# Desperodoo/distributed_multi_agent_reinforcement_learning

Measured on AMD Instinct MI355X. Metric: env-steps/sec (whole node), pursuit-evasion 8-agent 4096-env, higher is better.
Workload: dtype f64 environment / f32 policy (f32 matrix products evaluated from exact 3-way bf16 operand splits, f32 accumulation and storage)

## Files before the change

### distributed_multi_agent_reinforcement_learning_amd/csrc/mappo_ops.hip

```cpp
#include <hip/hip_runtime.h>
#include <stdint.h>
#include <stdlib.h>
#include <string.h>

#include <mutex>

#include "mappo_ops.h"
#include "mappo_ops_diag.h"
#include "sb_common.hpp"

namespace {

constexpr int MAX_P = 16;

__device__ __forceinline__ float msg_dot4(const float *w, const float4 &qv) {
    return __builtin_fmaf(w[3], qv.w, __builtin_fmaf(w[2], qv.z, __builtin_fmaf(w[1], qv.y, w[0] * qv.x)));
}

struct MsgDims {
    int R, P, K, E, din, q_div, adj_mode, rpb;
    int64_t p_rs, q_rs, e_rs, adj_rs, o_is;
};

__device__ __forceinline__ float rl_f(float v, int lane) { return __int_as_float(__builtin_amdgcn_readlane(__float_as_int(v), lane)); }
__device__ __forceinline__ uint32_t rl_u(uint32_t v, int lane) { return (uint32_t)__builtin_amdgcn_readlane((int)v, lane); }

struct MsgRow {
    float vp, ve, vq;
    uint32_t va0, va1;
    int kv;
};

template <bool QS, bool AS>
__device__ __forceinline__ MsgRow msgw_load(const MsgDims &d, int r, const float *__restrict__ p, const float *__restrict__ q,
                                            const float *__restrict__ e, const void *__restrict__ adj, const int32_t *__restrict__ kvalid,
                                            bool use_kvalid) {
    const int lane = threadIdx.x & 63, qr = r / d.q_div;
    MsgRow m;
    m.vp = lane < 4 * d.P ? p[(size_t)r * d.p_rs + lane] : 0.f;
    m.ve = (d.din == 8 && lane < 4) ? e[(size_t)r * d.e_rs + lane] : 0.f;
    m.vq = 0.f;
    if (QS) m.vq = lane < 4 * d.K ? q[(size_t)qr * d.q_rs + lane] : 0.f;
    m.va0 = m.va1 = 0u;
    if (AS) {
        if (d.adj_mode == MO_ADJ_TENSOR) {
            m.va0 = lane < d.P * d.K ? __float_as_uint(((const float *)adj)[(size_t)r * d.adj_rs + lane]) : 0u;
        } else if (d.adj_mode == MO_ADJ_BITS) {
            const uint32_t *bw = (const uint32_t *)adj + (size_t)r * d.adj_rs;
            const int n = d.P * MO_ADJ_ROW_WORDS(d.K);
            m.va0 = lane < n ? bw[lane] : 0u;
            m.va1 = lane + 64 < n ? bw[lane + 64] : 0u;
        }
    }
    m.kv = use_kvalid ? kvalid[qr] : d.K;
    return m;
}

template <bool QS>
__device__ __forceinline__ float4 msgw_q(const MsgRow &m, const float4 *__restrict__ q4, int j) {
    if (QS) return make_float4(rl_f(m.vq, 4 * j), rl_f(m.vq, 4 * j + 1), rl_f(m.vq, 4 * j + 2), rl_f(m.vq, 4 * j + 3));
    return q4[j];
}
template <bool AS>
__device__ __forceinline__ uint32_t msgw_word(const MsgRow &m, const uint32_t *__restrict__ bw, int idx) {
    if (AS) return idx < 64 ? rl_u(m.va0, idx) : rl_u(m.va1, idx - 64);
    return bw[idx];
}

struct MsgMask { uint64_t nz, col; bool zero_one; };
__device__ __forceinline__ MsgMask msgw_mask(const MsgRow &m, int P, int K) {
    const float a = __uint_as_float(m.va0);
    MsgMask k;
    k.nz = __ballot(a != 0.f);
    k.zero_one = __ballot(a != 0.f && a != 1.f) == 0ull;
    k.col = 0ull;
    for (int i = 0; i < P; i++) k.col |= 1ull << (i * K);
    return k;
}
__device__ __forceinline__ float msgw_row_norm(const MsgRow &m, const MsgMask &k, int i, int K) {
    if (k.zero_one) return (float)__popcll((k.nz >> (i * K)) & ((K >= 64) ? ~0ull : ((1ull << K) - 1ull)));
    float s = 0.f;
    for (int j = 0; j < K; j++) s += fabsf(__uint_as_float(rl_u(m.va0, i * K + j)));
    return s;
}

template <int EV>
struct FV {
    float v[EV];
    __device__ __forceinline__ FV() {}
    __device__ __forceinline__ FV(float s) {
#pragma unroll
        for (int e = 0; e < EV; e++) v[e] = s;
// ... 1671 lines not shown
    constexpr int U = 4;
    const int wave = threadIdx.x >> 6, lane = threadIdx.x & 63;
    const int i = lane & 15, kk = lane >> 4;
    const int m0 = blockIdx.y * 128 * AM + (wave >> 1) * 64 * AM, n0 = blockIdx.z * 128 * BN + (wave & 1) * 64 * BN;
    const int64_t steps = K >> 2;
    const int64_t s_beg = steps * blockIdx.x / gridDim.x, s_end = steps * (blockIdx.x + 1) / gridDim.x;
    const int64_t lda4 = 4 * lda, ldb4 = 4 * ldb;
    const float *pa = A + (4 * s_beg + kk) * lda + m0 + 4 * i;
    const float *pb = B + (4 * s_beg + kk) * ldb + n0 + 4 * i;
    v4f acc[AM][4][BN][4];
#pragma unroll
    for (int a = 0; a < AM; a++)
#pragma unroll
        for (int t = 0; t < 4; t++)
#pragma unroll
            for (int b = 0; b < BN; b++)
#pragma unroll
                for (int v = 0; v < 4; v++) acc[a][t][b][v] = (v4f){0.f, 0.f, 0.f, 0.f};
    const int64_t n_s = s_end - s_beg, pairs = n_s / (2 * U);
    WgradRegs<AM, BN, U> r0, r1;
    if (pairs > 0) wgrad_load<AM, BN, U>(r0, pa, pb, lda4, ldb4);
    for (int64_t c = 0; c < pairs; c++) {
        wgrad_load<AM, BN, U>(r1, pa + U * lda4, pb + U * ldb4, lda4, ldb4);
        __builtin_amdgcn_sched_barrier(0);
        wgrad_mma<AM, BN, U>(r0, acc);
        __builtin_amdgcn_sched_barrier(0);
        const int64_t adv = (c + 1 < pairs) ? 2 * U : U;
        pa += adv * lda4;
        pb += adv * ldb4;
        wgrad_load<AM, BN, U>(r0, pa, pb, lda4, ldb4);
        __builtin_amdgcn_sched_barrier(0);
        wgrad_mma<AM, BN, U>(r1, acc);
        __builtin_amdgcn_sched_barrier(0);
    }
    {
        pa = A + (4 * (s_beg + pairs * 2 * U) + kk) * lda + m0 + 4 * i;
        pb = B + (4 * (s_beg + pairs * 2 * U) + kk) * ldb + n0 + 4 * i;
        WgradRegs<AM, BN, 1> r;
        for (int64_t s = s_beg + pairs * 2 * U; s < s_end; s++) {
            wgrad_load<AM, BN, 1>(r, pa, pb, lda4, ldb4);
            wgrad_mma<AM, BN, 1>(r, acc);
            pa += lda4;
            pb += ldb4;
        }
        if (blockIdx.x == gridDim.x - 1 && (K & 3)) {
            const bool live = 4 * steps + kk < K;
#pragma unroll
            for (int a = 0; a < AM; a++) r.a[0][a] = live ? *(const float4 *)(pa + a * 64) : make_float4(0.f, 0.f, 0.f, 0.f);
#pragma unroll
            for (int b = 0; b < BN; b++) r.b[0][b] = live ? *(const float4 *)(pb + b * 64) : make_float4(0.f, 0.f, 0.f, 0.f);
            wgrad_mma<AM, BN, 1>(r, acc);
        }
    }
    float *po = part + ((size_t)blockIdx.x * M + m0 + 16 * kk) * N + n0 + 4 * i;
#pragma unroll
    for (int a = 0; a < AM; a++)
#pragma unroll
        for (int t = 0; t < 4; t++)
#pragma unroll
            for (int q = 0; q < 4; q++)
#pragma unroll
                for (int b = 0; b < BN; b++)
                    *(float4 *)(po + (size_t)(64 * a + 4 * q + t) * N + 64 * b) =
                        make_float4(acc[a][t][b][0][q], acc[a][t][b][1][q], acc[a][t][b][2][q], acc[a][t][b][3][q]);
}

__global__ __launch_bounds__(256) void k_wgrad_reduce(int S, int MN, const float *__restrict__ part, float *__restrict__ C, int accumulate) {
    __shared__ float sm[4][64];
    const int q = threadIdx.x >> 6, lane = threadIdx.x & 63;
    const int idx = blockIdx.x * 64 + lane;
    float s = 0.f;
    if (idx < MN) {
#pragma unroll 8
        for (int x = q; x < S; x += 4) s += part[(size_t)x * MN + idx];
    }
    sm[q][lane] = s;
    __syncthreads();
    if (q == 0 && idx < MN) {
        const float t = (sm[0][lane] + sm[1][lane]) + (sm[2][lane] + sm[3][lane]);
        C[idx] = accumulate ? C[idx] + t : t;
    }
}

constexpr int SB_DEPTH = 4;

template <int MT, int NT>
struct SbWgCfg {
    static constexpr int M = 128 * MT, N = 128 * NT, COLS = M + N, FQ = COLS / 4;
    static constexpr int CR = 16, NO = 2;
    static constexpr int WGM = MT >= NT ? 4 : 2;
    static constexpr int WGN = 8 / WGM;
    static constexpr int TM = M / 32 / WGM, TN = N / 32 / WGN;
    static constexpr int UNITS = 2 * NO * FQ;
    static constexpr int IMG = 3 * NO * COLS;
    static constexpr int LDS_BYTES = 2 * IMG * 16;
};

__device__ __forceinline__ int sb_swz(int f) { return (f & ~3) | ((f & 3) ^ ((f >> 3) & 3)); }
template <int MT, int NT>
__global__ __launch_bounds__(512) void k_sb_wgrad(const float *__restrict__ A, int64_t lda, const float *__restrict__ B, int64_t ldb, int64_t K,
                                                  float *__restrict__ part, const float *__restrict__ A2, int64_t lda2, int M1) {
    using C = SbWgCfg<MT, NT>;
    extern __shared__ uint4 sb_lds[];
    const int tid = threadIdx.x, lane = tid & 63, wave = tid >> 6;
    const int i = lane & 31, g = lane >> 5;
    const bool on = tid < C::UNITS;
    const int rest = on ? tid / C::FQ : 0, col = 4 * (tid % C::FQ);
    const int row_in_chunk = 4 * rest;
    const bool in_a2 = A2 != nullptr && col >= M1 && col < C::M;
    const int64_t ld = in_a2 ? lda2 : (col < C::M ? lda : ldb);
    const float *src = (in_a2 ? A2 + (col - M1) : (col < C::M ? A + col : B + (col - C::M))) + row_in_chunk * ld;
    const int slot2 = 2 * ((rest >> 1) * C::COLS + col) + (rest & 1), sx = (col >> 3) & 3;
    const int wm = wave / C::WGN, wn = wave % C::WGN;
    const int64_t chunks = K / C::CR;
    const int64_t c_beg = chunks * blockIdx.x / gridDim.x, c_end = chunks * (blockIdx.x + 1) / gridDim.x;

    f32x16 acc[C::TM][C::TN];
#pragma unroll
    for (int a = 0; a < C::TM; a++)
#pragma unroll
        for (int b = 0; b < C::TN; b++)
#pragma unroll
            for (int r = 0; r < 16; r++) acc[a][b][r] = 0.f;

    float4 raw[SB_DEPTH][4];
    auto fetch = [&](float4 (&r)[4], int64_t c) {
        if (!on || c >= c_end) return;
        const float *p = src + c * C::CR * ld;
#pragma unroll
        for (int j = 0; j < 4; j++) r[j] = *(const float4 *)(p + j * ld);
    };
    auto stage = [&](const float4 (&r)[4], uint4 *img) {
        if (!on) return;
        uint2 *img2 = (uint2 *)img;
#pragma unroll
        for (int t = 0; t < 4; t++) {
            uint32_t p[3][2];
#pragma unroll
            for (int q = 0; q < 2; q++) {
                const float x0 = t == 0 ? r[2 * q].x : t == 1 ? r[2 * q].y : t == 2 ? r[2 * q].z : r[2 * q].w;
                const float x1 = t == 0 ? r[2 * q + 1].x : t == 1 ? r[2 * q + 1].y : t == 2 ? r[2 * q + 1].z : r[2 * q + 1].w;
                sb_split2(x0, x1, p[0][q], p[1][q], p[2][q]);
            }
#pragma unroll
            for (int s = 0; s < 3; s++) img2[2 * s * C::NO * C::COLS + slot2 + 2 * (t ^ sx)] = make_uint2(p[s][0], p[s][1]);
        }
    };
    auto multiply = [&](const uint4 *buf) {
        const uint4 *img = buf + g * C::COLS;
        constexpr int PS = C::NO * C::COLS;
        if constexpr (C::TN <= C::TM) {
            uint4 b[C::TN][3];
#pragma unroll
            for (int nt = 0; nt < C::TN; nt++) {
                const int f = sb_swz(C::M + 32 * (wn * C::TN + nt) + i);
#pragma unroll
                for (int s = 0; s < 3; s++) b[nt][s] = img[s * PS + f];
            }
#pragma unroll
            for (int mt = 0; mt < C::TM; mt++) {
                const int f = sb_swz(32 * (wm * C::TM + mt) + i);
                uint4 a[3];
#pragma unroll
                for (int s = 0; s < 3; s++) a[s] = img[s * PS + f];
#pragma unroll
                for (int nt = 0; nt < C::TN; nt++) acc[mt][nt] = sb_mma6_32(a, b[nt], acc[mt][nt]);
            }
        } else {
            uint4 a[C::TM][3];
#pragma unroll
            for (int mt = 0; mt < C::TM; mt++) {
                const int f = sb_swz(32 * (wm * C::TM + mt) + i);
#pragma unroll
                for (int s = 0; s < 3; s++) a[mt][s] = img[s * PS + f];
            }
#pragma unroll
            for (int nt = 0; nt < C::TN; nt++) {
                const int f = sb_swz(C::M + 32 * (wn * C::TN + nt) + i);
                uint4 b[3];
#pragma unroll
                for (int s = 0; s < 3; s++) b[s] = img[s * PS + f];
#pragma unroll
                for (int mt = 0; mt < C::TM; mt++) acc[mt][nt] = sb_mma6_32(a[mt], b, acc[mt][nt]);
            }
        }
    };
#pragma unroll
    for (int d = 0; d < SB_DEPTH; d++) fetch(raw[d], c_beg + d);
    if (c_beg < c_end) {
        stage(raw[0], sb_lds);
        fetch(raw[0], c_beg + SB_DEPTH);
    }
    lds_barrier();
    for (int64_t c = c_beg; c < c_end; c += SB_DEPTH) {
#pragma unroll
        for (int d = 0; d < SB_DEPTH; d++) {
            const int64_t cc = c + d;
            if (cc >= c_end) break;
            uint4 *cur = sb_lds + (d & 1) * C::IMG, *nxt = sb_lds + ((d + 1) & 1) * C::IMG;
            if (wave < 4) {
                if (cc + 1 < c_end) stage(raw[(d + 1) % SB_DEPTH], nxt);
                fetch(raw[(d + 1) % SB_DEPTH], cc + 1 + SB_DEPTH);
                multiply(cur);
            } else {
                multiply(cur);
                if (cc + 1 < c_end) stage(raw[(d + 1) % SB_DEPTH], nxt);
                fetch(raw[(d + 1) % SB_DEPTH], cc + 1 + SB_DEPTH);
            }
            lds_barrier();
        }
    }
    if (blockIdx.x == gridDim.x - 1 && (K % C::CR)) {
        float4 r[4];
#pragma unroll
        for (int j = 0; j < 4; j++)
            r[j] = (on && chunks * C::CR + row_in_chunk + j < K) ? *(const float4 *)(src + (chunks * C::CR + j) * ld) : make_float4(0.f, 0.f, 0.f, 0.f);
        stage(r, sb_lds);
        lds_barrier();
        multiply(sb_lds);
    }
    float *po = part + (size_t)blockIdx.x * C::M * C::N + (size_t)(32 * wm * C::TM + 4 * g) * C::N + 32 * wn * C::TN + i;
#pragma unroll
    for (int mt = 0; mt < C::TM; mt++)
#pragma unroll
        for (int r = 0; r < 16; r++)
#pragma unroll
            for (int nt = 0; nt < C::TN; nt++) po[(size_t)(32 * mt + 8 * (r / 4) + (r % 4)) * C::N + 32 * nt] = acc[mt][nt][r];
}


struct NbrArgs {
    int R, P, E, T, relu;
    int64_t za_es, za_ts, zc_es, zc_ts;
    int64_t adj_rs;
    int64_t out_ld;
};
struct NbrJobs { mo_nbr_job j[MO_NBR_MAX_JOBS]; };
template <int PT>
__global__ void k_nbr_mean(NbrArgs a, NbrJobs jobs, const float *__restrict__ adj) {
    const mo_nbr_job &job = jobs.j[blockIdx.y];
    const float *__restrict__ za = job.z_actor, *__restrict__ zc = job.z_critic, *__restrict__ bias = job.bias;
    float *__restrict__ out_a = job.out_actor, *__restrict__ out_c = job.out_critic;
    const int P = a.P, E = a.E, f = threadIdx.x, lane = threadIdx.x & 63;
    const float bf = bias ? bias[f] : 0.f;
    const float inv_p = 1.f / fmaxf((float)P, 1e-12f);
    for (int r = blockIdx.x; r < a.R; r += gridDim.x) {
        const int n = r / a.T, t = r - n * a.T;
        if (out_a) {
            const float *zr = za + (size_t)n * a.za_es + (size_t)t * a.za_ts;
            float z[PT];
#pragma unroll
            for (int j = 0; j < PT; j++) z[j] = j < P ? zr[(size_t)j * E + f] : 0.f;
            float w = 0.f;
            if (P * P <= 64) {
                const float av = lane < P * P ? adj[(size_t)r * a.adj_rs + lane] : 0.f;
                const int li = lane / P < P ? lane / P : P - 1;
                float nrm = 0.f;
                for (int j = 0; j < P; j++) nrm += fabsf(__shfl(av, li * P + j));
                w = av / fmaxf(nrm, 1e-12f);
            }
#pragma unroll
            for (int i = 0; i < PT; i++)
                if (i < P) {
                    float acc = 0.f;
                    if (P * P <= 64) {
#pragma unroll
                        for (int j = 0; j < PT; j++)
                            if (j < P) acc = __builtin_fmaf(rl_f(w, i * P + j), z[j], acc);
                    } else {
                        const float *ar = adj + (size_t)r * a.adj_rs + (size_t)i * P;
                        float nrm = 0.f;
                        for (int j = 0; j < P; j++) nrm += fabsf(ar[j]);
                        nrm = fmaxf(nrm, 1e-12f);
#pragma unroll
                        for (int j = 0; j < PT; j++)
                            if (j < P) acc = __builtin_fmaf(ar[j] / nrm, z[j], acc);
                    }
                    acc += bf;
                    out_a[((size_t)r * P + i) * a.out_ld + f] = a.relu ? fmaxf(acc, 0.f) : acc;
                }
        }
        if (out_c) {
            const float *zr = zc + (size_t)n * a.zc_es + (size_t)t * a.zc_ts;
            float acc = 0.f;
#pragma unroll
            for (int j = 0; j < PT; j++)
                if (j < P) acc = __builtin_fmaf(inv_p, zr[(size_t)j * E + f], acc);
            acc += bf;
            acc = a.relu ? fmaxf(acc, 0.f) : acc;
            for (int i = 0; i < P; i++) out_c[((size_t)r * P + i) * a.out_ld + f] = acc;
        }
    }
}

__global__ __launch_bounds__(256) void k_nbr_mean4(NbrArgs a, NbrJobs jobs, const float *__restrict__ adj) {
    const mo_nbr_job &job = jobs.j[blockIdx.y];
    const float *__restrict__ za = job.z_actor, *__restrict__ zc = job.z_critic;
    float *__restrict__ out_a = job.out_actor, *__restrict__ out_c = job.out_critic;
    const int P = a.P, lane = threadIdx.x & 63, q = lane & 31, hf = lane >> 5;
    constexpr int E = 128;
    const float4 b4 = job.bias ? *(const float4 *)(job.bias + 4 * q) : make_float4(0.f, 0.f, 0.f, 0.f);
    const float inv_p = 1.f / fmaxf((float)P, 1e-12f);
    const bool relu = a.relu != 0;
    auto put = [&](float *dst, float4 v) {
        v.x += b4.x; v.y += b4.y; v.z += b4.z; v.w += b4.w;
        if (relu) { v.x = fmaxf(v.x, 0.f); v.y = fmaxf(v.y, 0.f); v.z = fmaxf(v.z, 0.f); v.w = fmaxf(v.w, 0.f); }
        *(float4 *)dst = v;
    };
    for (int r = blockIdx.x * 4 + (threadIdx.x >> 6); r < a.R; r += gridDim.x * 4) {
        const int n = r / a.T, t = r - n * a.T;
        if (out_a) {
// ... 138 lines not shown
            cs[k] += sk;
        }
    }
    float *dst = part + (size_t)blockIdx.x * ((NS + 1) * F + NS);
#pragma unroll
    for (int k = 0; k < NS; k++) dst[k * F + f] = acc[k];
    dst[NS * F + f] = cx;
    if (f == 0) {
#pragma unroll
        for (int k = 0; k < NS; k++) dst[(NS + 1) * F + k] = cs[k];
    }
}

__global__ void k_skinny_reduce(int nblk, int NS, int F, const float *__restrict__ part, int transposed, float *__restrict__ C,
                                float *__restrict__ colsum_x, float *__restrict__ colsum_s) {
    const int idx = blockIdx.x * (blockDim.x >> 6) + (threadIdx.x >> 6);
    const int lane = threadIdx.x & 63, per = (NS + 1) * F + NS;
    if (idx >= per) return;
    double s = 0.0;
    for (int b = lane; b < nblk; b += 64) s += (double)part[(size_t)b * per + idx];
    for (int off = 32; off > 0; off >>= 1) s += __shfl_xor(s, off);
    if (lane != 0) return;
    if (idx < NS * F) {
        const int k = idx / F, f = idx - k * F;
        C[transposed ? (size_t)f * NS + k : (size_t)k * F + f] = (float)s;
    } else if (idx < (NS + 1) * F) {
        if (colsum_x) colsum_x[idx - NS * F] = (float)s;
    } else if (colsum_s) {
        colsum_s[idx - (NS + 1) * F] = (float)s;
    }
}

int wgrad_split(int M, int N, int *am, int *bn) {
    *am = (M == 384 && N == 128) ? 3 : 1;
    *bn = (M == 128 && N == 384) ? 3 : 1;
    const int tiles = (M / (128 * *am)) * (N / (128 * *bn));
    int S = 256 / tiles;
    return S < 1 ? 1 : S;
}

int launch_msgw3(const mo_msg_rel *rel, int R, int P, int E, const float *p, int64_t p_rs, const int32_t *kvalid2, float *out, float *out_c,
                 int c_valid, int64_t out_stride, void *stream, bool pair, const float *Wp = nullptr, int64_t wp_rs = 0, const float *bp = nullptr,
                 float *pos_a = nullptr, float *pos_c = nullptr, int64_t pos_ld = 0, int c_rel2 = 1) {
    MsgDims d[3];
    int grid = 1;
    for (int r = 0; r < 3; r++) {
        const mo_msg_rel &m = rel[r];
        int rc = check_msg(R, P, m.K, E, m.din, m.q_div, m.adj_mode, m.adj, m.kvalid, m.e);
        if (rc) return rc;
        if ((m.q_rs & 3) || out_stride < 3 * E) return MO_ERR_BAD_ARG;
        if (r < 2 && m.adj_mode == MO_ADJ_VALID) return MO_ERR_BAD_ARG;
        d[r] = msg_dims(R, P, m.K, E, m.din, m.q_div, m.adj_mode, p_rs, m.q_rs, m.e_rs, m.adj_rs, out_stride, FWD_BLOCKS, &grid);
    }
    const bool s01 = msg_q_small(rel[0].K) && msg_q_small(rel[1].K) && msg_adj_small(P, rel[0].K, rel[0].adj_mode) &&
                     msg_adj_small(P, rel[1].K, rel[1].adj_mode);
    const bool as2 = msg_adj_small(P, rel[2].K, rel[2].adj_mode), ev2 = (E % 128) == 0;
    const bool halves = R <= 2048 && P > 4;
    const int pt = halves ? (P <= 8 ? 4 : 8) : (P <= 8 ? 8 : 16), gy = (P + pt - 1) / pt;
#define MSGW3_LAUNCH1(PT, S01, AS2, EV)                                                                                                     \
    hipLaunchKernelGGL((k_msgw3_fwd<PT, S01, AS2, EV>), dim3(grid, gy), dim3(E / EV), 0, (hipStream_t)stream, d[0], d[1], d[2], p, rel[0].q,   \
                       rel[0].e, rel[0].adj, rel[0].W, rel[0].b, rel[1].q, rel[1].adj, rel[1].W, rel[1].b, rel[2].q, rel[2].adj, kvalid2,      \
                       rel[2].W, rel[2].b, out, out_c, c_valid, c_rel2, Wp, wp_rs, bp, pos_a, pos_c, pos_ld ? pos_ld : (int64_t)E)
#define MSGW3_LAUNCH(PT, S01, AS2) do { if (ev2) MSGW3_LAUNCH1(PT, S01, AS2, 2); else MSGW3_LAUNCH1(PT, S01, AS2, 1); } while (0)
#define MSGW3_PT(PT) { if (s01 && as2) MSGW3_LAUNCH(PT, true, true); else if (s01) MSGW3_LAUNCH(PT, true, false); else if (as2) MSGW3_LAUNCH(PT, false, true); else MSGW3_LAUNCH(PT, false, false); }
    if (pt == 4) MSGW3_PT(4) else if (pt == 8) MSGW3_PT(8) else MSGW3_PT(16)
#undef MSGW3_PT
#undef MSGW3_LAUNCH
#undef MSGW3_LAUNCH1
    return (int)hipGetLastError();
}

}

constexpr int SB_WGRAD_WGS = 256;

static bool sb_wgrad_shape_ok(int M, int N) {
    return (M == 128 || M == 256 || M == 384) && (N == 128 || N == 256 || N == 384) && M + N <= 512 && M * N < 256 * 256;
}

template <int MT, int NT>
int launch_sb_wgrad(int64_t K, const float *A, int64_t lda, const float *B, int64_t ldb, float *Cm, int accumulate, float *part, hipStream_t st,
                    const float *A2 = nullptr, int64_t lda2 = 0, int M1 = 0) {
    using C = SbWgCfg<MT, NT>;
    static_assert(C::UNITS <= 512 && C::WGM * C::WGN == 8 && C::TM * C::WGM * 32 == C::M && C::TN * C::WGN * 32 == C::N && SB_DEPTH % 2 == 0, "tiling");
    static std::once_flag once;
    static hipError_t attr_rc = hipSuccess;
    std::call_once(once, [] { attr_rc = hipFuncSetAttribute((const void *)k_sb_wgrad<MT, NT>, hipFuncAttributeMaxDynamicSharedMemorySize, C::LDS_BYTES); });
    if (attr_rc != hipSuccess) return (int)attr_rc;
    hipLaunchKernelGGL((k_sb_wgrad<MT, NT>), dim3(SB_WGRAD_WGS), dim3(512), C::LDS_BYTES, st, A, lda, B, ldb, K, part, A2, lda2, M1);
    hipLaunchKernelGGL(k_wgrad_reduce, dim3((C::M * C::N + 63) / 64), dim3(256), 0, st, SB_WGRAD_WGS, C::M * C::N, (const float *)part, Cm, accumulate);
    return (int)hipGetLastError();
}

extern "C" {

int dhgn_msg_agg_fwd(int32_t R, int32_t P, int32_t K, int32_t E, int32_t din, const float *p, int64_t p_rs, const float *q,
                     int64_t q_rs, int32_t q_div, const float *e, int64_t e_rs, const void *adj, int64_t adj_rs, int32_t adj_mode,
                     const int32_t *kvalid, const float *W, const float *b, float *out, int64_t out_stride, void *stream) {
    int rc = check_msg(R, P, K, E, din, q_div, adj_mode, adj, kvalid, e);
    if (rc) return rc;
    if (R == 0) return 0;
    if ((q_rs & 3) || out_stride < E) return MO_ERR_BAD_ARG;
    int grid;
    const MsgDims d = msg_dims(R, P, K, E, din, q_div, adj_mode, p_rs, q_rs, e_rs, adj_rs, out_stride, FWD_BLOCKS, &grid);
    const bool qs = msg_q_small(K), as = msg_adj_small(P, K, adj_mode), ev2 = (E % 128) == 0;
#define MSGW_FWD1(PT, QS, AS, EV) hipLaunchKernelGGL((k_msgw_fwd<PT, QS, AS, EV>), dim3(grid), dim3(E / EV), 0, (hipStream_t)stream, d, p, q, e, adj, kvalid, W, b, out)
#define MSGW_FWD(PT, QS, AS) do { if (ev2) MSGW_FWD1(PT, QS, AS, 2); else MSGW_FWD1(PT, QS, AS, 1); } while (0)
#define MSGW_FWD_PT(PT) { if (qs && as) MSGW_FWD(PT, true, true); else if (qs) MSGW_FWD(PT, true, false); else if (as) MSGW_FWD(PT, false, true); else MSGW_FWD(PT, false, false); }
    if (P <= 8) MSGW_FWD_PT(8) else MSGW_FWD_PT(16)
#undef MSGW_FWD_PT
#undef MSGW_FWD
#undef MSGW_FWD1
    return (int)hipGetLastError();
}

int dhgn_msg_agg3_fwd(const mo_msg_rel *rel, int32_t R, int32_t P, int32_t E, const float *p, int64_t p_rs, float *out, int64_t out_stride,
                      void *stream) {
    if (!rel || !p || !out || R < 0) return MO_ERR_BAD_ARG;
    if (R == 0) return 0;
    return launch_msgw3(rel, R, P, E, p, p_rs, rel[2].kvalid, out, nullptr, 0, out_stride, stream, false);
}

int dhgn_msg_agg3_pair_fwd(const mo_msg_rel *rel, int32_t R, int32_t P, int32_t E, const float *p, int64_t p_rs, const int32_t *o_kvalid,
                           float *out_actor, float *out_critic, int64_t out_stride, void *stream) {
    if (!rel || !p || !out_actor || !out_critic || R < 0) return MO_ERR_BAD_ARG;
    if (R == 0) return 0;
    for (int r = 0; r < 3; r++)
        if (rel[r].adj_mode != MO_ADJ_TENSOR && rel[r].adj_mode != MO_ADJ_BITS) return MO_ERR_BAD_ARG;
    return launch_msgw3(rel, R, P, E, p, p_rs, o_kvalid, out_actor, out_critic, o_kvalid != nullptr, out_stride, stream, true);
}

int dhgn_msg_agg3_pair01_fwd(const mo_msg_rel *rel, int32_t R, int32_t P, int32_t E, const float *p, int64_t p_rs, float *out_actor,
                             float *out_critic, int64_t out_stride, void *stream) {
    if (!rel || !p || !out_actor || !out_critic || R < 0) return MO_ERR_BAD_ARG;
    if (R == 0) return 0;
    for (int r = 0; r < 3; r++)
        if (rel[r].adj_mode != MO_ADJ_TENSOR && rel[r].adj_mode != MO_ADJ_BITS) return MO_ERR_BAD_ARG;
    return launch_msgw3(rel, R, P, E, p, p_rs, nullptr, out_actor, out_critic, 0, out_stride, stream, true, nullptr, 0, nullptr, nullptr, nullptr, 0, 0);
}

int dhgn_msg_agg3_pair_pos_fwd(const mo_msg_rel *rel, int32_t R, int32_t P, int32_t E, const float *p, int64_t p_rs, const int32_t *o_kvalid,
                               float *out_actor, float *out_critic, int64_t out_stride, const float *Wp, int64_t wp_row_stride, const float *bp,
                               float *pos_actor, float *pos_critic, int64_t pos_stride, void *stream) {
    if (!rel || !p || !out_actor || !out_critic || R < 0 || !Wp || !bp || !pos_actor || wp_row_stride < 4 || pos_stride < E) return MO_ERR_BAD_ARG;
    if (R == 0) return 0;
    for (int r = 0; r < 3; r++)
        if (rel[r].adj_mode != MO_ADJ_TENSOR && rel[r].adj_mode != MO_ADJ_BITS) return MO_ERR_BAD_ARG;
    return launch_msgw3(rel, R, P, E, p, p_rs, o_kvalid, out_actor, out_critic, o_kvalid != nullptr, out_stride, stream, true, Wp, wp_row_stride, bp,
                        pos_actor, pos_critic, pos_stride);
}

int64_t dhgn_msg_agg_bwd_workspace(int32_t E, int32_t din) { return (int64_t)BWD_BLOCKS * (din + 1) * E * sizeof(float); }

static int msg_agg_bwd_launch(int32_t R, int32_t P, int32_t K, int32_t E, int32_t din, const float *p, int64_t p_rs, const float *q,
                              int64_t q_rs, int32_t q_div, const float *e, int64_t e_rs, const void *adj, int64_t adj_rs, int32_t adj_mode,
                              const int32_t *kvalid, const float *W, const float *b, const float *gout, const float *gout_c, int64_t gout_stride,
                              float *dW, float *db, void *workspace, void *stream) {
    int rc = check_msg(R, P, K, E, din, q_div, adj_mode, adj, kvalid, e);
    if (rc) return rc;
    if (!workspace || !gout || !dW || !db) return MO_ERR_BAD_ARG;
    if ((q_rs & 3) || gout_stride < E) return MO_ERR_BAD_ARG;
    if (gout_c && adj_mode != MO_ADJ_TENSOR) return MO_ERR_BAD_ARG;
    int grid;
    const MsgDims d = msg_dims(R, P, K, E, din, q_div, adj_mode, p_rs, q_rs, e_rs, adj_rs, gout_stride, BWD_BLOCKS, &grid);
    const bool qs = msg_q_small(K), as = msg_adj_small(P, K, adj_mode), ev2 = (E % 128) == 0;
#define MSGW_BWD2(PT, QS, AS, EV, PAIR) \
    hipLaunchKernelGGL((k_msgw_bwd<PT, QS, AS, EV, PAIR>), dim3(grid), dim3(E / EV), 0, (hipStream_t)stream, d, p, q, e, adj, kvalid, W, b, gout, gout_c, (float *)workspace)
#define MSGW_BWD1(PT, QS, AS, EV) do { if (gout_c) MSGW_BWD2(PT, QS, AS, EV, true); else MSGW_BWD2(PT, QS, AS, EV, false); } while (0)
#define MSGW_BWD(PT, QS, AS) do { if (ev2) MSGW_BWD1(PT, QS, AS, 2); else MSGW_BWD1(PT, QS, AS, 1); } while (0)
#define MSGW_BWD_PT(PT) { if (qs && as) MSGW_BWD(PT, true, true); else if (qs) MSGW_BWD(PT, true, false); else if (as) MSGW_BWD(PT, false, true); else MSGW_BWD(PT, false, false); }
    if (P <= 8) MSGW_BWD_PT(8) else MSGW_BWD_PT(16)
#undef MSGW_BWD_PT
// ... 463 lines not shown
```

Baseline: 2.606 million.

## Warp-specialize weight-gradient kernel into dedicated loader and MMA waves

Splits the split-bf16 weight-gradient GEMM kernel into 4 producer waves that fetch, split and stage operands into double-buffered LDS, and 8 consumer waves that only issue matrix-core multiplies. Before, all 8 waves interleaved staging and MMA work. The aim is to overlap global loads and bf16 splitting with MFMA work and to lower register pressure in the MMA waves. In exchange the block grows to 768 threads, loaders may cover several units each with a reduced prefetch depth, and the kernel moves into a separate header.

```diff
diff --git a/distributed_multi_agent_reinforcement_learning_amd/csrc/mappo_ops.hip b/distributed_multi_agent_reinforcement_learning_amd/csrc/mappo_ops.hip
--- a/distributed_multi_agent_reinforcement_learning_amd/csrc/mappo_ops.hip
+++ b/distributed_multi_agent_reinforcement_learning_amd/csrc/mappo_ops.hip
@@ -8,6 +8,7 @@
 #include "mappo_ops.h"
 #include "mappo_ops_diag.h"
 #include "sb_common.hpp"
+#include "sb_wgrad.hpp"
 
 namespace {
 
@@ -1845,151 +1846,6 @@
     }
 }
 
-constexpr int SB_DEPTH = 4;
-
-template <int MT, int NT>
-struct SbWgCfg {
-    static constexpr int M = 128 * MT, N = 128 * NT, COLS = M + N, FQ = COLS / 4;
-    static constexpr int CR = 16, NO = 2;
-    static constexpr int WGM = MT >= NT ? 4 : 2;
-    static constexpr int WGN = 8 / WGM;
-    static constexpr int TM = M / 32 / WGM, TN = N / 32 / WGN;
-    static constexpr int UNITS = 2 * NO * FQ;
-    static constexpr int IMG = 3 * NO * COLS;
-    static constexpr int LDS_BYTES = 2 * IMG * 16;
-};
-
-__device__ __forceinline__ int sb_swz(int f) { return (f & ~3) | ((f & 3) ^ ((f >> 3) & 3)); }
-template <int MT, int NT>
-__global__ __launch_bounds__(512) void k_sb_wgrad(const float *__restrict__ A, int64_t lda, const float *__restrict__ B, int64_t ldb, int64_t K,
-                                                  float *__restrict__ part, const float *__restrict__ A2, int64_t lda2, int M1) {
-    using C = SbWgCfg<MT, NT>;
-    extern __shared__ uint4 sb_lds[];
-    const int tid = threadIdx.x, lane = tid & 63, wave = tid >> 6;
-    const int i = lane & 31, g = lane >> 5;
-    const bool on = tid < C::UNITS;
-    const int rest = on ? tid / C::FQ : 0, col = 4 * (tid % C::FQ);
-    const int row_in_chunk = 4 * rest;
-    const bool in_a2 = A2 != nullptr && col >= M1 && col < C::M;
-    const int64_t ld = in_a2 ? lda2 : (col < C::M ? lda : ldb);
-    const float *src = (in_a2 ? A2 + (col - M1) : (col < C::M ? A + col : B + (col - C::M))) + row_in_chunk * ld;
-    const int slot2 = 2 * ((rest >> 1) * C::COLS + col) + (rest & 1), sx = (col >> 3) & 3;
-    const int wm = wave / C::WGN, wn = wave % C::WGN;
-    const int64_t chunks = K / C::CR;
-    const int64_t c_beg = chunks * blockIdx.x / gridDim.x, c_end = chunks * (blockIdx.x + 1) / gridDim.x;
-
-    f32x16 acc[C::TM][C::TN];
-#pragma unroll
-    for (int a = 0; a < C::TM; a++)
-#pragma unroll
-        for (int b = 0; b < C::TN; b++)
-#pragma unroll
-            for (int r = 0; r < 16; r++) acc[a][b][r] = 0.f;
-
-    float4 raw[SB_DEPTH][4];
-    auto fetch = [&](float4 (&r)[4], int64_t c) {
-        if (!on || c >= c_end) return;
-        const float *p = src + c * C::CR * ld;
-#pragma unroll
-        for (int j = 0; j < 4; j++) r[j] = *(const float4 *)(p + j * ld);
-    };
-    auto stage = [&](const float4 (&r)[4], uint4 *img) {
-        if (!on) return;
-        uint2 *img2 = (uint2 *)img;
-#pragma unroll
-        for (int t = 0; t < 4; t++) {
-            uint32_t p[3][2];
-#pragma unroll
-            for (int q = 0; q < 2; q++) {
-                const float x0 = t == 0 ? r[2 * q].x : t == 1 ? r[2 * q].y : t == 2 ? r[2 * q].z : r[2 * q].w;
-                const float x1 = t == 0 ? r[2 * q + 1].x : t == 1 ? r[2 * q + 1].y : t == 2 ? r[2 * q + 1].z : r[2 * q + 1].w;
-                sb_split2(x0, x1, p[0][q], p[1][q], p[2][q]);
-            }
-#pragma unroll
-            for (int s = 0; s < 3; s++) img2[2 * s * C::NO * C::COLS + slot2 + 2 * (t ^ sx)] = make_uint2(p[s][0], p[s][1]);
-        }
-    };
-    auto multiply = [&](const uint4 *buf) {
-        const uint4 *img = buf + g * C::COLS;
-        constexpr int PS = C::NO * C::COLS;
-        if constexpr (C::TN <= C::TM) {
-            uint4 b[C::TN][3];
-#pragma unroll
-            for (int nt = 0; nt < C::TN; nt++) {
-                const int f = sb_swz(C::M + 32 * (wn * C::TN + nt) + i);
-#pragma unroll
-                for (int s = 0; s < 3; s++) b[nt][s] = img[s * PS + f];
-            }
-#pragma unroll
-            for (int mt = 0; mt < C::TM; mt++) {
-                const int f = sb_swz(32 * (wm * C::TM + mt) + i);
-                uint4 a[3];
-#pragma unroll
-                for (int s = 0; s < 3; s++) a[s] = img[s * PS + f];
-#pragma unroll
-                for (int nt = 0; nt < C::TN; nt++) acc[mt][nt] = sb_mma6_32(a, b[nt], acc[mt][nt]);
-            }
-        } else {
-            uint4 a[C::TM][3];
-#pragma unroll
-            for (int mt = 0; mt < C::TM; mt++) {
-                const int f = sb_swz(32 * (wm * C::TM + mt) + i);
-#pragma unroll
-                for (int s = 0; s < 3; s++) a[mt][s] = img[s * PS + f];
-            }
-#pragma unroll
-            for (int nt = 0; nt < C::TN; nt++) {
-                const int f = sb_swz(C::M + 32 * (wn * C::TN + nt) + i);
-                uint4 b[3];
-#pragma unroll
-                for (int s = 0; s < 3; s++) b[s] = img[s * PS + f];
-#pragma unroll
-                for (int mt = 0; mt < C::TM; mt++) acc[mt][nt] = sb_mma6_32(a[mt], b, acc[mt][nt]);
-            }
-        }
-    };
-#pragma unroll
-    for (int d = 0; d < SB_DEPTH; d++) fetch(raw[d], c_beg + d);
-    if (c_beg < c_end) {
-        stage(raw[0], sb_lds);
-        fetch(raw[0], c_beg + SB_DEPTH);
-    }
-    lds_barrier();
-    for (int64_t c = c_beg; c < c_end; c += SB_DEPTH) {
-#pragma unroll
-        for (int d = 0; d < SB_DEPTH; d++) {
-            const int64_t cc = c + d;
-            if (cc >= c_end) break;
-            uint4 *cur = sb_lds + (d & 1) * C::IMG, *nxt = sb_lds + ((d + 1) & 1) * C::IMG;
-            if (wave < 4) {
-                if (cc + 1 < c_end) stage(raw[(d + 1) % SB_DEPTH], nxt);
-                fetch(raw[(d + 1) % SB_DEPTH], cc + 1 + SB_DEPTH);
-                multiply(cur);
-            } else {
-                multiply(cur);
-                if (cc + 1 < c_end) stage(raw[(d + 1) % SB_DEPTH], nxt);
-                fetch(raw[(d + 1) % SB_DEPTH], cc + 1 + SB_DEPTH);
-            }
-            lds_barrier();
-        }
-    }
-    if (blockIdx.x == gridDim.x - 1 && (K % C::CR)) {
-        float4 r[4];
-#pragma unroll
-        for (int j = 0; j < 4; j++)
-            r[j] = (on && chunks * C::CR + row_in_chunk + j < K) ? *(const float4 *)(src + (chunks * C::CR + j) * ld) : make_float4(0.f, 0.f, 0.f, 0.f);
-        stage(r, sb_lds);
-        lds_barrier();
-        multiply(sb_lds);
-    }
-    float *po = part + (size_t)blockIdx.x * C::M * C::N + (size_t)(32 * wm * C::TM + 4 * g) * C::N + 32 * wn * C::TN + i;
-#pragma unroll
-    for (int mt = 0; mt < C::TM; mt++)
-#pragma unroll
-        for (int r = 0; r < 16; r++)
-#pragma unroll
-            for (int nt = 0; nt < C::TN; nt++) po[(size_t)(32 * mt + 8 * (r / 4) + (r % 4)) * C::N + 32 * nt] = acc[mt][nt][r];
-}
 
 
 struct NbrArgs {
@@ -2294,12 +2150,11 @@
 int launch_sb_wgrad(int64_t K, const float *A, int64_t lda, const float *B, int64_t ldb, float *Cm, int accumulate, float *part, hipStream_t st,
                     const float *A2 = nullptr, int64_t lda2 = 0, int M1 = 0) {
     using C = SbWgCfg<MT, NT>;
-    static_assert(C::UNITS <= 512 && C::WGM * C::WGN == 8 && C::TM * C::WGM * 32 == C::M && C::TN * C::WGN * 32 == C::N && SB_DEPTH % 2 == 0, "tiling");
     static std::once_flag once;
     static hipError_t attr_rc = hipSuccess;
     std::call_once(once, [] { attr_rc = hipFuncSetAttribute((const void *)k_sb_wgrad<MT, NT>, hipFuncAttributeMaxDynamicSharedMemorySize, C::LDS_BYTES); });
     if (attr_rc != hipSuccess) return (int)attr_rc;
-    hipLaunchKernelGGL((k_sb_wgrad<MT, NT>), dim3(SB_WGRAD_WGS), dim3(512), C::LDS_BYTES, st, A, lda, B, ldb, K, part, A2, lda2, M1);
+    hipLaunchKernelGGL((k_sb_wgrad<MT, NT>), dim3(SB_WGRAD_WGS), dim3(SB_WG_THREADS), C::LDS_BYTES, st, A, lda, B, ldb, K, part, A2, lda2, M1);
     hipLaunchKernelGGL(k_wgrad_reduce, dim3((C::M * C::N + 63) / 64), dim3(256), 0, st, SB_WGRAD_WGS, C::M * C::N, (const float *)part, Cm, accumulate);
     return (int)hipGetLastError();
 }
diff --git a/distributed_multi_agent_reinforcement_learning_amd/csrc/sb_wgrad.hpp b/distributed_multi_agent_reinforcement_learning_amd/csrc/sb_wgrad.hpp
--- /dev/null
+++ b/distributed_multi_agent_reinforcement_learning_amd/csrc/sb_wgrad.hpp
@@ -0,0 +1,190 @@
+#pragma once
+#include "sb_common.hpp"
+
+constexpr int SB_WG_MMA_WAVES = 8, SB_WG_LOAD_WAVES = 4, SB_WG_THREADS = 64 * (SB_WG_MMA_WAVES + SB_WG_LOAD_WAVES);
+
+template <int MT, int NT>
+struct SbWgCfg {
+    static constexpr int M = 128 * MT, N = 128 * NT, COLS = M + N, FQ = COLS / 4;
+    static constexpr int CR = 16, NO = 2;
+    static constexpr int WGM = MT >= NT ? 4 : 2;
+    static constexpr int WGN = 8 / WGM;
+    static constexpr int TM = M / 32 / WGM, TN = N / 32 / WGN;
+    static constexpr int UNITS = 2 * NO * FQ;
+    static constexpr int LT = 64 * SB_WG_LOAD_WAVES;
+    static constexpr int UL = (UNITS + LT - 1) / LT;
+    static constexpr int DEPTH = UL == 1 ? 4 : 3;
+    static constexpr int IMG = 3 * NO * COLS;
+    static constexpr int LDS_BYTES = 2 * IMG * 16;
+};
+
+__device__ __forceinline__ int sb_swz(int f) { return (f & ~3) | ((f & 3) ^ ((f >> 3) & 3)); }
+
+template <int MT, int NT>
+__device__ __forceinline__ void sb_wgrad_loader(int lw, int lane, const float *__restrict__ A, int64_t lda, const float *__restrict__ B, int64_t ldb, int64_t K,
+                                                const float *__restrict__ A2, int64_t lda2, int M1, int64_t c_beg, int64_t c_end, bool tail,
+                                                uint4 *sb_lds) {
+    using C = SbWgCfg<MT, NT>;
+    const float *src[C::UL];
+    int64_t ld[C::UL];
+    bool on[C::UL];
+    int row_in_chunk[C::UL], slot2[C::UL], sx[C::UL];
+#pragma unroll
+    for (int u = 0; u < C::UL; u++) {
+        const int unit = 64 * lw + lane + C::LT * u;
+        on[u] = (u + 1) * C::LT <= C::UNITS || 64 * lw + C::LT * u < C::UNITS;
+        const int rest = on[u] ? unit / C::FQ : 0, col = on[u] ? 4 * (unit % C::FQ) : 0;
+        row_in_chunk[u] = 4 * rest;
+        const bool in_a2 = A2 != nullptr && col >= M1 && col < C::M;
+        ld[u] = in_a2 ? lda2 : (col < C::M ? lda : ldb);
+        src[u] = (in_a2 ? A2 + (col - M1) : (col < C::M ? A + col : B + (col - C::M))) + row_in_chunk[u] * ld[u];
+        slot2[u] = 2 * ((rest >> 1) * C::COLS + col) + (rest & 1);
+        sx[u] = (col >> 3) & 3;
+    }
+    constexpr int D = C::DEPTH;
+    float4 raw[D][C::UL][4];
+    auto fetch = [&](float4 (&r)[C::UL][4], int64_t c) {
+        c = c < c_end ? c : c_end - 1;
+#pragma unroll
+        for (int u = 0; u < C::UL; u++) {
+            const float *p = src[u] + c * C::CR * ld[u];
+#pragma unroll
+            for (int j = 0; j < 4; j++) r[u][j] = *(const float4 *)(p + j * ld[u]);
+        }
+    };
+    auto stage = [&](const float4 (&r)[C::UL][4], uint4 *img) {
+        uint2 *img2 = (uint2 *)img;
+#pragma unroll
+        for (int u = 0; u < C::UL; u++) {
+            if (!on[u]) continue;
+#pragma unroll
+            for (int t = 0; t < 4; t++) {
+                uint32_t p[3][2];
+#pragma unroll
+                for (int q = 0; q < 2; q++) {
+                    const float4 &v0 = r[u][2 * q], &v1 = r[u][2 * q + 1];
+                    const float x0 = t == 0 ? v0.x : t == 1 ? v0.y : t == 2 ? v0.z : v0.w;
+                    const float x1 = t == 0 ? v1.x : t == 1 ? v1.y : t == 2 ? v1.z : v1.w;
+                    sb_split2(x0, x1, p[0][q], p[1][q], p[2][q]);
+                }
+#pragma unroll
+                for (int s = 0; s < 3; s++) img2[2 * s * C::NO * C::COLS + slot2[u] + 2 * (t ^ sx[u])] = make_uint2(p[s][0], p[s][1]);
+            }
+        }
+    };
+    if (c_beg < c_end) {
+#pragma unroll
+        for (int d = 0; d < D; d++) fetch(raw[d], c_beg + d);
+        __builtin_amdgcn_sched_barrier(0);
+        stage(raw[0], sb_lds);
+        __builtin_amdgcn_sched_barrier(0);
+        fetch(raw[0], c_beg + D);
+    }
+    lds_barrier();
+    for (int64_t c = c_beg; c < c_end; c += D) {
+#pragma unroll
+        for (int d = 0; d < D; d++) {
+            const int64_t cc = c + d;
+            if (cc >= c_end) break;
+            stage(raw[(d + 1) % D], sb_lds + ((cc + 1 - c_beg) & 1) * C::IMG);
+            fetch(raw[(d + 1) % D], cc + 1 + D);
+            lds_barrier();
+        }
+    }
+    if (tail) {
+        const int64_t r0 = (K / C::CR) * C::CR;
+        float4 r[C::UL][4];
+#pragma unroll
+        for (int u = 0; u < C::UL; u++)
+#pragma unroll
+            for (int j = 0; j < 4; j++)
+                r[u][j] = (on[u] && r0 + row_in_chunk[u] + j < K) ? *(const float4 *)(src[u] + (r0 + j) * ld[u]) : make_float4(0.f, 0.f, 0.f, 0.f);
+        stage(r, sb_lds);
+        lds_barrier();
+    }
+}
+
+template <int MT, int NT>
+__device__ __forceinline__ void sb_wgrad_mma(int wave, int lane, int64_t c_beg, int64_t c_end, bool tail, const uint4 *sb_lds, float *__restrict__ part) {
+    using C = SbWgCfg<MT, NT>;
+    const int i = lane & 31, g = lane >> 5;
+    const int wm = wave / C::WGN, wn = wave % C::WGN;
+    f32x16 acc[C::TM][C::TN];
+#pragma unroll
+    for (int a = 0; a < C::TM; a++)
+#pragma unroll
+        for (int b = 0; b < C::TN; b++)
+#pragma unroll
+            for (int r = 0; r < 16; r++) acc[a][b][r] = 0.f;
+    auto multiply = [&](const uint4 *buf) {
+        const uint4 *img = buf + g * C::COLS;
+        constexpr int PS = C::NO * C::COLS;
+        if constexpr (C::TN <= C::TM) {
+            uint4 b[C::TN][3];
+#pragma unroll
+            for (int nt = 0; nt < C::TN; nt++) {
+                const int f = sb_swz(C::M + 32 * (wn * C::TN + nt) + i);
+#pragma unroll
+                for (int s = 0; s < 3; s++) b[nt][s] = img[s * PS + f];
+            }
+#pragma unroll
+            for (int mt = 0; mt < C::TM; mt++) {
+                const int f = sb_swz(32 * (wm * C::TM + mt) + i);
+                uint4 a[3];
+#pragma unroll
+                for (int s = 0; s < 3; s++) a[s] = img[s * PS + f];
+#pragma unroll
+                for (int nt = 0; nt < C::TN; nt++) acc[mt][nt] = sb_mma6_32(a, b[nt], acc[mt][nt]);
+            }
+        } else {
+            uint4 a[C::TM][3];
+#pragma unroll
+            for (int mt = 0; mt < C::TM; mt++) {
+                const int f = sb_swz(32 * (wm * C::TM + mt) + i);
+#pragma unroll
+                for (int s = 0; s < 3; s++) a[mt][s] = img[s * PS + f];
+            }
+#pragma unroll
+            for (int nt = 0; nt < C::TN; nt++) {
+                const int f = sb_swz(C::M + 32 * (wn * C::TN + nt) + i);
+                uint4 b[3];
+#pragma unroll
+                for (int s = 0; s < 3; s++) b[s] = img[s * PS + f];
+#pragma unroll
+                for (int mt = 0; mt < C::TM; mt++) acc[mt][nt] = sb_mma6_32(a[mt], b, acc[mt][nt]);
+            }
+        }
+    };
+    lds_barrier();
+    for (int64_t c = c_beg; c < c_end; c++) {
+        multiply(sb_lds + ((c - c_beg) & 1) * C::IMG);
+        lds_barrier();
+    }
+    if (tail) {
+        lds_barrier();
+        multiply(sb_lds);
+    }
+    float *po = part + (size_t)blockIdx.x * C::M * C::N + (size_t)(32 * wm * C::TM + 4 * g) * C::N + 32 * wn * C::TN + i;
+#pragma unroll
+    for (int mt = 0; mt < C::TM; mt++)
+#pragma unroll
+        for (int r = 0; r < 16; r++)
+#pragma unroll
+            for (int nt = 0; nt < C::TN; nt++) po[(size_t)(32 * mt + 8 * (r / 4) + (r % 4)) * C::N + 32 * nt] = acc[mt][nt][r];
+}
+
+template <int MT, int NT>
+__global__ __launch_bounds__(SB_WG_THREADS) void k_sb_wgrad(const float *__restrict__ A, int64_t lda, const float *__restrict__ B, int64_t ldb, int64_t K,
+                                                            float *__restrict__ part, const float *__restrict__ A2, int64_t lda2, int M1) {
+    using C = SbWgCfg<MT, NT>;
+    static_assert(C::WGM * C::WGN == SB_WG_MMA_WAVES && C::TM * C::WGM * 32 == C::M && C::TN * C::WGN * 32 == C::N, "tiling");
+    extern __shared__ uint4 sb_lds[];
+    const int wave = __builtin_amdgcn_readfirstlane(threadIdx.x >> 6);
+    const int64_t chunks = K / C::CR;
+    const int64_t c_beg = chunks * blockIdx.x / gridDim.x, c_end = chunks * (blockIdx.x + 1) / gridDim.x;
+    const bool tail = blockIdx.x == gridDim.x - 1 && (K % C::CR);
+    if (wave >= SB_WG_MMA_WAVES)
+        sb_wgrad_loader<MT, NT>(wave - SB_WG_MMA_WAVES, threadIdx.x & 63, A, lda, B, ldb, K, A2, lda2, M1, c_beg, c_end, tail, sb_lds);
+    else
+        sb_wgrad_mma<MT, NT>(wave, threadIdx.x & 63, c_beg, c_end, tail, sb_lds, part);
+}
```

Result: faster. 2.646 million, median of 6 (+1.6%).
